# JihyongOh/DeMFI

Measured on AMD Instinct MI355X. Metric: interpolated frames/sec @720p x8 MFI (N_tst=3), higher is better.
Workload: dtype f16; 1 GPU; DeMFI-Net_rb N_tst=3, x8 MFI, 720x1280 (padded 736x1280), fp16, clip-parallel windows, random-init weights; uint8 frames host->HBM->host inside the timed region (PNG codec excluded), 8 distinct windows; graph=True, parallelism=clip1, n_ctx=7, n_trunk=3

## Files before the change

### demfi_amd/_lib.py

```python
import ctypes as C
import os

_HERE = os.path.dirname(os.path.abspath(__file__))
LIB_PATH = os.environ.get('DEMFI_HIP_LIB') or os.path.join(_HERE, 'csrc', 'libdemfi_hip.so')

F16, F32 = 0, 1
ABI_VERSION = 8
ACT_NONE, ACT_RELU, ACT_TANH, ACT_SIGMOID = 0, 1, 2, 3
MODE_STORE, MODE_MUL, MODE_GRU = 0, 1, 2
BT601, BT709 = 0, 1
SITING_420JPEG, SITING_420MPEG2 = 0, 1
YUV_LAYOUT = {'420': 0, '422': 1, '444': 2, 'mono': 3}
OWNERS = ('sep', 'wstream7', 'ws2', 'wstream3', 'c64', 'narrow_nhwc', 'narrow_thin', 'general')
OWNERS_COUT_PERM = frozenset(range(6))
MAX_PIECES, MAX_CHUNKS, MAX_SEGS, MAX_OCTS = 48, 40, 8, 32


class View(C.Structure):
    _fields_ = [('ptr', C.c_void_p), ('sx', C.c_int64), ('sy', C.c_int64), ('sc', C.c_int64), ('sb', C.c_int64),
                ('is_f32', C.c_int32), ('_pad', C.c_int32)]


class Piece(C.Structure):
    _fields_ = [('v', View), ('nch', C.c_int32), ('lds_ch', C.c_int32), ('up_shift', C.c_int32), ('fat', C.c_int32)]


class Chunk(C.Structure):
    _fields_ = [('first_piece', C.c_int32), ('n_pieces', C.c_int32), ('nks', C.c_int32), ('_pad', C.c_int32),
                ('w_off', C.c_int64)]


class Seg(C.Structure):
# ... 39 lines not shown


class Op(C.Structure):
    _fields_ = [('kind', C.c_int32), ('conv', C.c_int32), ('nch', C.c_int32), ('_pad', C.c_int32), ('macs', C.c_int64),
                ('a', View), ('b', View), ('o', View), ('p', C.c_void_p * 32), ('t', C.c_void_p), ('name', C.c_char * 64),
                ('bt', Batch)]


_SIGS = {
    'demfi_abi_version': (C.c_int, []),
    'demfi_last_error': (C.c_char_p, []),
    'demfi_device_info': (C.c_int, [C.c_char_p, C.c_int, C.POINTER(C.c_int), C.POINTER(C.c_int64)]),
    'demfi_pack_conv_weights': (C.c_int, [C.c_void_p, C.c_int, C.c_int, C.c_int, C.c_int, C.c_void_p, C.c_int,
                                          C.c_void_p, C.c_int, C.c_void_p, C.c_int, C.c_int, C.c_int, C.c_void_p,
                                          C.POINTER(C.c_int64)]),
    'demfi_conv_lds_bytes': (C.c_int64, [C.POINTER(Conv)]),
    'demfi_conv2d': (C.c_int, [C.POINTER(Conv), C.c_void_p, C.c_void_p]),
    'demfi_resblock_eligible': (C.c_int, [C.POINTER(Conv), C.POINTER(Conv)]),
    'demfi_resblock3x3_c64': (C.c_int, [C.POINTER(Conv), C.POINTER(Conv), C.c_void_p]),
    'demfi_gru_r_eligible': (C.c_int, [C.POINTER(Conv)]),
    'demfi_gru_r': (C.c_int, [C.POINTER(Conv), C.c_void_p]),
    'demfi_gru_zq_eligible': (C.c_int, [C.POINTER(Conv), C.POINTER(Conv)]),
    'demfi_gru_zq': (C.c_int, [C.POINTER(Conv), C.POINTER(Conv), C.c_void_p]),
    'demfi_space_to_depth': (C.c_int, [C.c_void_p, C.c_void_p, C.c_int, C.c_int, C.c_int, C.c_void_p]),
    'demfi_reflect_pad': (C.c_int, [C.c_void_p, C.c_void_p, C.c_int, C.c_int, C.c_int, C.c_int, C.c_int, C.c_void_p]),
    'demfi_overlay_mean': (C.c_int, [C.c_void_p, C.c_void_p, C.c_int, C.c_int, C.c_void_p]),
    'demfi_cfr_workspace_bytes': (C.c_int64, [C.c_int, C.c_int]),
    'demfi_cfr_reset': (C.c_int, [C.c_void_p, C.c_int, C.c_int, C.c_void_p]),
    'demfi_cfr_flow_align': (C.c_int, [C.c_void_p, C.c_void_p, C.c_void_p, C.c_int, C.c_int, C.c_void_p, C.c_void_p,
                                       C.c_void_p, C.c_void_p]),
    'demfi_warp_blend': (C.c_int, [C.POINTER(View), C.c_void_p, C.POINTER(View), C.c_void_p, C.c_void_p, C.c_void_p,
                                   C.POINTER(View), C.c_int, C.c_int, C.c_int, C.c_void_p, C.c_void_p, C.c_void_p]),
    'demfi_warp_blend_pack': (C.c_int, [C.POINTER(View), C.c_void_p, C.POINTER(View), C.c_void_p, C.c_void_p, C.c_void_p,
                                        C.POINTER(View), C.c_int, C.c_int, C.c_void_p, C.c_void_p, C.c_int, C.c_void_p]),
    'demfi_warp_blend_batched': (C.c_int, [C.POINTER(View), C.c_void_p, C.POINTER(View), C.c_void_p, C.c_void_p, C.c_void_p,
                                           C.POINTER(View), C.c_int, C.c_int, C.c_int, C.c_void_p, C.c_void_p, C.c_int, C.POINTER(Batch),
                                           C.c_void_p]),
    'demfi_cfr_flow_align_batched': (C.c_int, [C.c_void_p, C.c_void_p, C.c_void_p, C.c_int, C.c_int, C.c_void_p, C.c_void_p,
                                               C.POINTER(Batch), C.c_void_p]),
    'demfi_cfr_flow_align_pack': (C.c_int, [C.c_void_p, C.c_void_p, C.c_void_p, C.c_void_p, C.c_int, C.c_int, C.c_void_p, C.c_void_p, C.c_void_p,
                                            C.c_int, C.POINTER(Batch), C.c_void_p]),
    'demfi_pack_planes_batched': (C.c_int, [C.c_void_p, C.c_int, C.c_void_p, C.c_int, C.c_int64, C.c_int, C.c_int, C.POINTER(Batch),
                                            C.c_void_p]),
    'demfi_fgac_gather': (C.c_int, [C.POINTER(View), C.c_void_p, C.POINTER(View), C.c_int, C.c_int, C.c_int,
                                    C.c_void_p, C.c_void_p]),
    'demfi_fgac_window': (C.c_int, [C.POINTER(View), C.POINTER(View), C.c_void_p, C.POINTER(View), C.c_int, C.c_int, C.c_int,
# ... 146 lines not shown
```

### demfi_amd/csrc/conv_build.cpp

```cpp
#include "plan.h"
#include <algorithm>
#include <string.h>

namespace plan {

constexpr int64_t LDS_BUDGET = 78 * 1024;

int conv_shape(int dtype, int H, int W, int stride, int batch, const Layer& l, const demfi_conv_src* srcs, int n_srcs,
               const demfi_conv_dst* dsts, int n_dsts, ConvShape& out, const char* name, int pad_y, int pad_x, int grid_div)
{
    if (dtype != DEMFI_F16 && dtype != DEMFI_F32) return demfi_set_error(DEMFI_ERR_ARG, "%s: dtype", name);
    if (!srcs || !dsts || n_srcs <= 0 || n_dsts <= 0 || n_dsts > DEMFI_MAX_SEGS || (stride != 1 && stride != 2))
        return demfi_set_error(DEMFI_ERR_ARG, "%s: sources / destinations / stride", name);
    const int cout = l.cout, cin = l.cin, kh = l.kh, kw = l.kw;
    const int esz = dtype == DEMFI_F32 ? 4 : 2;
    const int64_t LH = 7 * stride + kh, LW = 31 * stride + kw;
    int n_oct = 0;
    for (int i = 0; i < n_dsts; ++i) n_oct += (dsts[i].n + 7) / 8;
    const int sub = (n_oct + 3) / 4;
    int nco = sub <= 5 ? sub : 4;
    int rec = 128;
    int src_nch = 0;
    for (int i = 0; i < n_srcs; ++i) src_nch += srcs[i].nch;
    const bool ws2_s2 = stride == 2 && kh == 4 && kw == 4, ws2_s1 = stride == 1 && kh == 3 && kw == 3 && src_nch > 64;
// ... 180 lines not shown
                pm[i] = cout_map[sb * 32 + (r >> 4) * 16 + ((r >> 2) & 1) * 8 + ((r >> 3) & 1) * 4 + (r & 3)];
            }
            cout_map.swap(pm);
        }
    }
    out.wbytes = d.w_blk_stride * 16 * (cout_pad / (32 * nco));
    return DEMFI_OK;
}

int conv_pack(const ConvShape& s, const Layer& l, const float* w, const float* bias, std::vector<uint8_t>& wpack, std::vector<float>& bias_packed)
{
    int64_t nbytes = 0;
    wpack.resize(s.wbytes);
    const int st = demfi_pack_conv_weights(w, l.cout, l.cin, l.kh, l.kw, s.cin_map.data(), (int)s.cin_map.size(), s.nks.data(), (int)s.nks.size(),
                                           s.cout_map.data(), s.d.cout_pad, s.d.nco, s.d.dtype, wpack.data(), &nbytes);
    if (st < 0) return st;
    if (nbytes != s.wbytes) return demfi_set_error(DEMFI_ERR_ARG, "conv_pack: %lld B packed, %lld B planned", (long long)nbytes, (long long)s.wbytes);
    bias_packed.assign(s.d.cout_pad, 0.0f);
    for (int i = 0; i < s.d.cout_pad; ++i)
        if (s.cout_map[i] >= 0 && bias) bias_packed[i] = bias[s.cout_map[i]];
    return DEMFI_OK;
}

}

extern "C" int demfi_conv_build(int dtype, int H, int W, int stride, int batch, const float* w, const float* bias, int cout, int cin,
                                int kh, int kw, const demfi_conv_src* srcs, int n_srcs, const demfi_conv_dst* dsts, int n_dsts,
                                demfi_conv* desc, void* wpack, int64_t* wpack_bytes, float* bias_packed, int32_t* cout_pad)
{
    if (!w || !desc || !wpack_bytes || !cout_pad || H <= 0 || W <= 0 || batch <= 0 || cout <= 0 || cin <= 0 || kh <= 0 || kw <= 0)
        return demfi_set_error(DEMFI_ERR_ARG, "demfi_conv_build: bad arguments");
    const plan::Layer l = {cout, cin, kh, kw};
    plan::ConvShape s;
    int st = plan::conv_shape(dtype, H, W, stride, batch, l, srcs, n_srcs, dsts, n_dsts, s, "demfi_conv_build");
    if (st < 0) return st;
    *cout_pad = s.d.cout_pad;
    *wpack_bytes = s.wbytes;
    *desc = s.d;
    if (!wpack) return DEMFI_OK;
    std::vector<uint8_t> wp;
    std::vector<float> bp;
    st = plan::conv_pack(s, l, w, bias, wp, bp);
    if (st < 0) return st;
    memcpy(wpack, wp.data(), wp.size());
    if (bias_packed) memcpy(bias_packed, bp.data(), bp.size() * 4);
    return DEMFI_OK;
// ... 2 lines not shown
```

### demfi_amd/csrc/conv_kernels.h

```cpp
#pragma once
#include <hip/hip_runtime.h>
#include "demfi_hip.h"

int demfi_conv_general_launch(const demfi_conv* h, const demfi_conv* dev, hipStream_t st, size_t lds);
int demfi_c64_launch(const demfi_conv* h, const demfi_conv* dev, hipStream_t st);
int demfi_narrow_launch(const demfi_conv* h, const demfi_conv* dev, hipStream_t st, bool thin);
bool demfi_sep_eligible(const demfi_conv* h);
int demfi_sep_launch(const demfi_conv* h, const demfi_conv* dev, hipStream_t st);
bool demfi_wstream_eligible(const demfi_conv* h, int ks = 7, int nch = 2);
int demfi_wstream_launch(const demfi_conv* h, const demfi_conv* dev, hipStream_t st);
int demfi_wstream3_launch(const demfi_conv* h, const demfi_conv* dev, hipStream_t st);
int demfi_c64_trace_collect(unsigned long long* acc);
int demfi_narrow_trace_collect(unsigned long long* acc);
int demfi_sep_trace_collect(unsigned long long* acc);
int demfi_wstream_trace_collect(unsigned long long* acc);
```

### demfi_amd/csrc/ctx.cpp

```cpp
#include "plan.h"
#include <stdlib.h>
#include <string.h>

using namespace plan;

namespace {

int run_ops(demfi_ctx* c, const OpList& ops, void* stream)
{
    for (const demfi_op& op : ops) {
        const int st = demfi_run_op(c, &op, stream);
        if (st < 0) return st;
    }
    return DEMFI_OK;
}

bool check_idx(const demfi_ctx* c, int trunk, int q)
{
    return c && trunk >= 0 && trunk < c->n_trunk && q >= 0 && q < c->n_ctx;
}

}

static int size_context(demfi_ctx* c, demfi_ctx** out)
{
    layer_table(c);
    compute_layout(c, 0, 0);
    int st = run_builder(c, true);
    if (st < 0) { delete c; return st; }
    static const bool arena_on = !(getenv("DEMFI_ARENA") && atoi(getenv("DEMFI_ARENA")) == 0);
    if (arena_on && !c->op_kind) {
        std::vector<const OpList*> per_t = {&c->head_ops[0][0]}, tr = {&c->tr_ops[0]}, none;
        for (int it = 0; it < c->N; ++it) per_t.push_back(&c->iter_ops[0][0][it]);
        std::vector<const OpList*> per_t_all = per_t;
        if (c->n_ctx > 1) { per_t_all.push_back(&c->tb_head_ops[0]); for (int it = 0; it < c->N; ++it) per_t_all.push_back(&c->tb_iter_ops[0][it]); }
        const ArenaPlan pt = plan_arena(c, c->t_bufs[0][0], c->n_ctx, per_t, none,
                                        {"Ft", "u1", "u2", "u3", "d0", "d1", "d2", "rF", "dec_a", "dec_t", "dec_b", "frec0", "frec1", "re1", "rd64", "de1",
                                         "bl1", "xb", "zb", "rh", "h1", "fo1", "g_a", "g_t", "g_b", "g_p2", "misc16", "ref16", "ref32", "agg3s"});
        const ArenaPlan ptr_ = plan_arena(c, c->tr_bufs[0], 0, tr, per_t_all,
                                          {"s2d", "f1", "x0", "grow", "gffcat", "g0", "g1", "up", "enc_a", "enc_t", "enc_b", "rk", "skk", "rkp", "skp",
                                           "smp", "E", "wg"});
        c->arena_t = pt;
        c->arena_tr = ptr_;
        if (getenv("DEMFI_ARENA_DEBUG")) {
            for (auto* pl : {&c->arena_t, &c->arena_tr}) {
                fprintf(stderr, "arena %s: %.1f MB\n", pl == &c->arena_t ? "per-t (all contexts)" : "trunk", pl->size / 1e6);
                for (auto& kv : pl->off) fprintf(stderr, "   %-8s at %.1f MB\n", kv.first.c_str(), kv.second / 1e6);
            }
        }
// ... 259 lines not shown
extern "C" int demfi_ctx_get_op(const demfi_ctx* c, int segment, int trunk, int q, int iter, int index, demfi_op* out)
{
    const OpList* o = seg_ops(c, segment, trunk, q, iter);
    if (!o || !out || index < 0 || index >= (int)o->size()) return demfi_set_error(DEMFI_ERR_ARG, "demfi_ctx_get_op: bad arguments");
    *out = (*o)[index];
    return DEMFI_OK;
}

extern "C" int demfi_ctx_num_convs(const demfi_ctx* c) { return c ? (int)c->descs.size() : 0; }

extern "C" const demfi_conv* demfi_ctx_conv_desc(const demfi_ctx* c, int index)
{
    if (!c || index < 0 || index >= (int)c->descs.size()) return nullptr;
    return &c->descs[index];
}

extern "C" int demfi_run_op(demfi_ctx* c, const demfi_op* op, void* stream)
{
    if (!c || !op || !c->bound || c->on_host) return demfi_set_error(DEMFI_ERR_ARG, "demfi_run_op: context not bound to device memory");
    const int H = c->H, W = c->W;
    switch (op->kind) {
    case DEMFI_OP_CONV:
        if (op->conv < 0 || op->conv >= (int)c->descs.size()) return demfi_set_error(DEMFI_ERR_ARG, "demfi_run_op: descriptor index");
        return demfi_conv2d(&c->descs[op->conv], (const demfi_conv*)(c->base + c->desc_off) + op->conv, stream);
    case DEMFI_OP_RESBLOCK:
        if (op->conv < 0 || op->conv >= (int)c->descs.size() || op->nch < 0 || op->nch >= (int)c->descs.size())
            return demfi_set_error(DEMFI_ERR_ARG, "demfi_run_op: descriptor index");
        return demfi_resblock3x3_c64(&c->descs[op->conv], &c->descs[op->nch], stream);
    case DEMFI_OP_GRU_R:
        if (op->conv < 0 || op->conv >= (int)c->descs.size()) return demfi_set_error(DEMFI_ERR_ARG, "demfi_run_op: descriptor index");
        return demfi_gru_r(&c->descs[op->conv], stream);
    case DEMFI_OP_GRU_ZQ:
        if (op->conv < 0 || op->conv >= (int)c->descs.size() || op->nch < 0 || op->nch >= (int)c->descs.size())
            return demfi_set_error(DEMFI_ERR_ARG, "demfi_run_op: descriptor index");
        return demfi_gru_zq(&c->descs[op->conv], &c->descs[op->nch], stream);
    case DEMFI_OP_PACK:
        if (op->bt.nb > 1)
            return demfi_pack_planes_batched((const float* const*)op->p, op->nch, op->o.ptr, c->dtype, op->o.sx, H, W, &op->bt, stream);
        return demfi_pack_planes((const float* const*)op->p, op->nch, op->o.ptr, c->dtype, op->o.sx, H, W, stream);
    case DEMFI_OP_VIZ:
        if (op->conv == 0) return demfi_absmean_map(&op->a, op->b.ptr ? &op->b : nullptr, (float*)op->p[0], op->nch, H, W, stream);
        if (op->conv == 1) return demfi_minmax_normalize((float*)op->p[0], (int64_t)H * W, (float*)op->p[1], stream);
        if (op->conv == 2) return demfi_one_minus((const float*)op->p[1], (float*)op->p[0], (int64_t)H * W, stream);
        return demfi_set_error(DEMFI_ERR_ARG, "demfi_run_op: visualisation sub-op %d", op->conv);
    case DEMFI_OP_S2D:
        return demfi_space_to_depth((const float*)op->p[0], (void*)op->p[1], c->dtype, H, W, stream);
// ... 32 lines not shown
```

### demfi_amd/csrc/plan.cpp

```cpp
#include "plan.h"
#include <algorithm>
#include <string.h>

namespace plan {

void layer_table(demfi_ctx* c)
{
    auto& t = c->table;
    if (c->op_kind == 1) {
        for (const char* g : {"z", "r", "q"}) t[std::string("conv") + g + "1"] = {64, 128, 1, 5};
        for (const char* g : {"z", "r", "q"}) t[std::string("conv") + g + "2"] = {64, 128, 5, 1};
        return;
    }
    if (c->op_kind == 2) {
        t["conv_ref_k"] = {64, 64, 1, 1}; t["conv_source_k"] = {64, 64, 1, 1}; t["fusion"] = {64, 64, 1, 1};
        t["w_gen"] = {64, 128, 3, 3}; t["w_gen_2"] = {1, 64, 3, 3};
        return;
    }
    const int nf = c->hp.nf, r2 = c->hp.scale_factor * c->hp.scale_factor;
    const int G0 = 96, G = 32, Cn = 4, D = 12;
    auto add = [&](const std::string& n, int cout, int cin, int kh, int kw) { t[n] = {cout, cin, kh, kw}; };
    std::string p = "FF_RDB_Module.";
    add(p + "SFENet1", G0, 12 * r2, 5, 5);
    add(p + "SFENet2", G0, G0, 3, 3);
// ... 611 lines not shown
                m2.insert(m2.end(), 7, -1);
                SubW wb = sub_weight(p + "enc1", sel, false);
                conv(th, p + "enc1#t", {fsrc(B["Ft"], 0), fsrc_map(B["misc16"], m2)},
                     {D(fview(B["u1"]), range(0, 64), R, DEMFI_MODE_STORE, fview(TB["u1a"]))}, H2, W2, ConvOpt().strided(2).weights(wb));
            } else
            conv(th, p + "enc1", {fsrc(aF, 0, 0, -1, 0), fsrc(aF, 64, 0, -1, 1), fsrc(B["Ft"], 128), fsrc_map(B["misc16"], m)},
                 {D(fview(B["u1"]), range(0, 64), R)}, H2, W2, ConvOpt().strided(2));
        }
        conv(th, p + "enc2", {fsrc(B["u1"], 0)}, {D(fview(B["u2"]), range(0, 128), R)}, H4, W4, ConvOpt().strided(2));
        conv(th, p + "enc3", {fsrc(B["u2"], 0)}, {D(fview(B["u3"]), range(0, 256), R)}, H8, W8, ConvOpt().strided(2));
        conv(th, p + "dec0", {fsrc(B["u3"], 0)}, {D(fview(B["d0"]), range(0, 256), R)}, H8, W8);
        conv(th, p + "dec1", {fsrc(B["d0"], 0, 0, -1, -1, 1), fsrc(B["u2"], 256)}, {D(fview(B["d1"]), range(0, 128), R)}, H4, W4);
        conv(th, p + "dec2", {fsrc(B["d1"], 0, 0, -1, -1, 1), fsrc(B["u1"], 128)}, {D(fview(B["d2"]), range(0, 64), R)}, H2, W2);
        if (c->dtype == DEMFI_F16) {
            Found f3;
            if (!lookup(p + "dec3", f3)) return;
            const Layer l3 = f3.l;
            auto phase_view = [&](demfi_view v, int dy, int dx) {
                const int64_t elt = v.is_f32 ? 4 : 2;
                v.ptr = (char*)v.ptr + ((int64_t)dy * v.sy + (int64_t)dx * v.sx) * elt;
                v.sx *= 2; v.sy *= 2;
                return v;
            };
            for (int dy = 0; dy < 2 && status >= 0; ++dy) {
                SubW wf2;
                wf2.shape = {10, l3.cin, 3, 3};
                for (int dx = 0; dx < 2 && status >= 0; ++dx) {
                    std::vector<float> w9e;
                    if (!dry) {
                        w9e.assign((size_t)l3.cout * l3.cin * 9, 0.0f);
                        for (int co = 0; co < l3.cout; ++co)
                            for (int ci = 0; ci < l3.cin; ++ci) {
                                const float* w9 = &(*f3.w)[((size_t)co * l3.cin + ci) * 9];
                                float* we = &w9e[((size_t)co * l3.cin + ci) * 9];
                                for (int ky = 0; ky < 3; ++ky)
                                    for (int kx = 0; kx < 3; ++kx) {
                                        const int a = dy == 0 ? (ky >= 1) : (ky >= 2), b = dx == 0 ? (kx >= 1) : (kx >= 2);
                                        we[(a + dy) * 3 + (b + dx)] += w9[ky * 3 + kx];
                                    }
                            }
                    }
                    const std::string nm = p + "dec3#p" + std::to_string(dy) + std::to_string(dx);
                    const Layer l9 = {l3.cout, l3.cin, 3, 3};
                    const SubW wa = rows(l9, &w9e, f3.b, 5, 64), wb = rows(l9, &w9e, f3.b, 69, 64), wf = rows(l9, &w9e, f3.b, 0, 5);
                    conv(th, nm + "a", {fsrc(B["d2"], 0)},
                         {D(phase_view(fview(B["rF"], 0, 0), dy, dx), range(0, 64), T, DEMFI_MODE_STORE, phase_view(fview(aF, 0, 0), dy, dx))},
                         H2, W2, ConvOpt().weights(wa));
                    conv(th, nm + "b", {fsrc(B["d2"], 0)},
                         {D(phase_view(fview(B["rF"], 0, 1), dy, dx), range(0, 64), T, DEMFI_MODE_STORE, phase_view(fview(aF, 0, 1), dy, dx))},
                         H2, W2, ConvOpt().weights(wb));
                    wf2.w.insert(wf2.w.end(), wf.w.begin(), wf.w.end());
                    wf2.b.insert(wf2.b.end(), wf.b.begin(), wf.b.end());
                }
                if (status >= 0) {
                    conv(th, p + "dec3#p" + std::to_string(dy) + "xf", {fsrc(B["d2"], 0)},
                         {D(phase_view(delta_v(0, 0), dy, 0), range(0, 4), DEMFI_ACT_NONE, DEMFI_MODE_STORE, phase_view(tview(B["ft"]), dy, 0)),
                          D(phase_view(delta_v(0, 4), dy, 0), {4}, DEMFI_ACT_NONE, DEMFI_MODE_STORE, phase_view(tview(ffo, 4), dy, 0)),
                          D(phase_view(delta_v(0, 0), dy, 1), range(5, 9), DEMFI_ACT_NONE, DEMFI_MODE_STORE, phase_view(tview(B["ft"]), dy, 1)),
                          D(phase_view(delta_v(0, 4), dy, 1), {9}, DEMFI_ACT_NONE, DEMFI_MODE_STORE, phase_view(tview(ffo, 4), dy, 1))},
                         H2, W2, ConvOpt().weights(wf2).packed(phase_view(fview(B["delta16"]), dy, 0), 0, 4, 16, 20));
                }
            }
        } else
        conv(th, p + "dec3", {fsrc(B["d2"], 0, 0, -1, -1, 1)},
             {D(fview(B["rF"], 0, 0), range(5, 69), T, DEMFI_MODE_STORE, fview(aF, 0, 0)),
              D(fview(B["rF"], 0, 1), range(69, 133), T, DEMFI_MODE_STORE, fview(aF, 0, 1)),
              D(delta_v(0, 0), range(0, 4), DEMFI_ACT_NONE, DEMFI_MODE_STORE, tview(B["ft"])),
              D(delta_v(0, 4), {4}, DEMFI_ACT_NONE, DEMFI_MODE_STORE, tview(ffo, 4))}, H, W);
        warp(th, "warp_fat", 64, fview(B["rF"], 0, 0), fview(B["rF"], 0, 1), fview(B["rF"], 0, 2), delta_p(0, 0), delta_p(0, 2),
             delta_p(0, 4), plane(B["occ"], 0), tp);
        conv(th, "Dec_first", {fsrc(B["rF"], 0)}, {D(fview(B["dec_a"]), range(0, 64), R)}, H, W, ConvOpt().batched(3));
        const Tensor* cur = resblocks(th, "Decoder_res", c->hp.num_resb_dec, B["dec_a"], B["dec_t"], B["dec_b"], H, W, 3);
        conv(th, "Dec_last1", {fsrc(*cur, 0)}, {D(fview(B["dec_t"]), range(0, 64), R)}, H, W, ConvOpt().batched(3));
// ... 158 lines not shown
```

### demfi_amd/csrc/plan.h

```cpp
#pragma once
#include "common.h"
#include <map>
#include <string>
#include <vector>

namespace plan {

struct Tensor {
    int64_t off = -1;
    int kind = 0;
    int d[4] = {0, 0, 0, 0};
    int64_t bytes = 0;
    int64_t cstride = 0;
    int id = 0;
};

struct ArenaPlan { std::map<std::string, int64_t> off; int64_t size = 0; int64_t cstride = 0; bool on = false; };

struct Weight { std::vector<float> data; std::vector<int64_t> shape; };

struct Layer { int cout, cin, kh, kw; };

typedef std::map<std::string, Tensor> BufSet;
typedef std::vector<demfi_op> OpList;

struct ConvShape {
    demfi_conv d;
    std::vector<int32_t> cin_map, cout_map, nks;
    int64_t wbytes = 0;
    int64_t macs = 0;
};

int conv_shape(int dtype, int H, int W, int stride, int batch, const Layer& l, const demfi_conv_src* srcs, int n_srcs,
               const demfi_conv_dst* dsts, int n_dsts, ConvShape& out, const char* name, int pad_y = -1, int pad_x = -1, int grid_div = 1);
int conv_pack(const ConvShape& s, const Layer& l, const float* w, const float* bias, std::vector<uint8_t>& wpack, std::vector<float>& bias_packed);

}

struct demfi_ctx {
    int H, W, N, dtype, n_trunk, n_ctx;
    int op_kind = 0, op_batch = 1;
    demfi_hparams hp;
    std::map<std::string, plan::Weight> weights;
    std::map<std::string, plan::Layer> table;
    int64_t w_region = 0, w_bytes = 0, desc_off = 0, zero_off = 0, total = 0, n_descs = 0;
    std::vector<plan::BufSet> tr_bufs;
    std::vector<std::vector<plan::BufSet>> t_bufs;
    std::vector<int64_t> id_cstride;
    plan::ArenaPlan arena_t, arena_tr;
    bool bound = false, on_host = false;
    char* base = nullptr;
    std::vector<demfi_conv> descs;
    std::vector<plan::OpList> tr_ops;
    std::vector<std::vector<plan::OpList>> head_ops;
    std::vector<std::vector<std::vector<plan::OpList>>> iter_ops;
    std::vector<plan::OpList> tb_head_ops;
    std::vector<std::vector<plan::OpList>> tb_iter_ops;
    std::vector<std::string> fused_dry, fused_now;
    std::vector<uint8_t> host_blob;
    std::map<std::string, std::pair<int64_t, int64_t>> pack_cache;
    int64_t blob_fill = 0;
};

// ... 12 lines not shown
```

### demfi_amd/engine.py

```python
import ctypes as C

import numpy as np
import torch

from . import _lib as L
from .spec import HyperParams


def _np_f32(t):
    return np.ascontiguousarray(t.detach().to('cpu', torch.float32).numpy())


class _Src:
    __slots__ = ('fat', 'ptr', 'sx', 'sy', 'sc', 'sb', 'is_f32', 'cin', 'up')

    def __init__(self, fat, ptr, sx, sy, sc, sb, is_f32, cin, up=0):
        self.fat, self.ptr, self.sx, self.sy, self.sc, self.sb = fat, ptr, sx, sy, sc, sb
        self.is_f32, self.cin, self.up = is_f32, list(cin), up


class _Dst:
    __slots__ = ('view', 'couts', 'act', 'mode', 'res', 'aux', 'scale', 'dy', 'dx')

    def __init__(self, view, couts, act=L.ACT_NONE, mode=L.MODE_STORE, res=None, aux=None, scale=1, dy=0, dx=0):
# ... 121 lines not shown
            host[off:off + a.nbytes] = a.reshape(-1)
        self.weight_blob = torch.from_numpy(host).to(self.device)
        self._wblobs = None
        base = self.weight_blob.data_ptr()
        self.zero_page = torch.zeros(256, dtype=torch.uint8, device=self.device)
        self._keep.append(self.zero_page)
        for d in self._descs:
            d.wpack = base + (d.wpack or 0)
            d.bias = base + (d.bias or 0)
            d.zero_page = self.zero_page.data_ptr()
        sz = C.sizeof(L.Conv)
        raw = bytearray(len(self._descs) * sz)
        for i, d in enumerate(self._descs):
            raw[i * sz:(i + 1) * sz] = bytes(d)
        self.desc_dev = torch.frombuffer(raw, dtype=torch.uint8).clone().to(self.device)
        self._desc_sz = sz

    def launch_conv(self, i, stream, what='conv'):
        L.check(self.lib.demfi_conv2d(C.byref(self._descs[i]), self.desc_dev.data_ptr() + i * self._desc_sz, stream), what)

    def launch_resblock(self, i1, i2, stream, what='resblock'):
        L.check(self.lib.demfi_resblock3x3_c64(C.byref(self._descs[i1]), C.byref(self._descs[i2]), stream), what)


    def launch_gru_r(self, i, stream, what='gru_r'):
        L.check(self.lib.demfi_gru_r(C.byref(self._descs[i]), stream), what)

    def launch_gru_zq(self, iz, iq, stream, what='gru_zq'):
        L.check(self.lib.demfi_gru_zq(C.byref(self._descs[iz]), C.byref(self._descs[iq]), stream), what)


SEG_TRUNK, SEG_HEAD, SEG_ITER, SEG_TB_HEAD, SEG_TB_ITER = 0, 1, 2, 3, 4
KIND_NAME = {0: 'conv', 1: 'pack', 2: 's2d', 3: 'overlay', 4: 'fgac', 5: 'gate', 6: 'cfr', 7: 'warp', 8: 'fgac_window', 9: 'avg_pool',
             10: 'resblock',
             11: 'gru_r', 12: 'gru_zq', 13: 'viz'}


class Engine:

    def __init__(self, state_dict, H, W, dtype=torch.float16, device='cuda:0', max_updates=3, hp=None, n_ctx=1, n_trunk=1):
        if H % 8 or W % 8:
            raise ValueError('DeMFI-Net needs H, W multiples of 8 (the harness pads to 32): got %dx%d' % (H, W))
        self.lib = L.load()
        self.H, self.W, self.N = H, W, max_updates
        self.dtype = dtype
        self.f32 = dtype == torch.float32
# ... 285 lines not shown
```

### include/demfi_hip.h

```cpp
#ifndef DEMFI_HIP_H
#define DEMFI_HIP_H

#include <stdint.h>

#ifdef __cplusplus
extern "C" {
#endif

#define DEMFI_ABI_VERSION 8

enum demfi_dtype { DEMFI_F16 = 0, DEMFI_F32 = 1 };

enum demfi_status {
    DEMFI_OK = 0,
    DEMFI_ERR_ARG = -1,
    DEMFI_ERR_HIP = -2,
    DEMFI_ERR_NODEV = -3
};

enum demfi_yuv_matrix { DEMFI_BT601 = 0, DEMFI_BT709 = 1 };
enum demfi_chroma_siting { DEMFI_420JPEG = 0, DEMFI_420MPEG2 = 1 };
enum demfi_yuv_layout { DEMFI_YUV_420 = 0, DEMFI_YUV_422 = 1, DEMFI_YUV_444 = 2, DEMFI_YUV_MONO = 3 };

enum demfi_act { DEMFI_ACT_NONE = 0, DEMFI_ACT_RELU = 1, DEMFI_ACT_TANH = 2, DEMFI_ACT_SIGMOID = 3 };
// ... 84 lines not shown
} demfi_u8_sink;

int         demfi_abi_version(void);
const char* demfi_last_error(void);
int         demfi_device_info(char* name, int len, int* n_cu, int64_t* hbm_bytes);

int demfi_pack_conv_weights(const float* w_oihw, int cout, int cin, int kh, int kw,
                            const int32_t* cin_map, int n_k, const int32_t* chunk_nks, int n_chunks,
                            const int32_t* cout_map, int cout_pad, int nco, int dtype,
                            void* out, int64_t* out_bytes);

int64_t demfi_conv_lds_bytes(const demfi_conv* host_desc);

int demfi_conv2d(const demfi_conv* host_desc, const demfi_conv* dev_desc, void* stream);

int demfi_resblock_eligible(const demfi_conv* h1, const demfi_conv* h2);
int demfi_resblock3x3_c64(const demfi_conv* h1, const demfi_conv* h2, void* stream);

int demfi_gru_r_eligible(const demfi_conv* hr);
int demfi_gru_r(const demfi_conv* hr, void* stream);
int demfi_gru_zq_eligible(const demfi_conv* hz, const demfi_conv* hq);
int demfi_gru_zq(const demfi_conv* hz, const demfi_conv* hq, void* stream);

int demfi_space_to_depth(const float* x, void* out, int dtype, int H, int W, void* stream);

int demfi_reflect_pad(const float* x, float* out, int planes, int h, int w, int H, int W, void* stream);

int demfi_overlay_mean(const float* x, float* out, int H, int W, void* stream);

int64_t demfi_cfr_workspace_bytes(int H, int W);
int demfi_cfr_reset(int64_t* acc, int H, int W, void* stream);
int demfi_cfr_flow_align(const float* flow01, const float* flow10, const float* t, int H, int W,
                         int64_t* acc, float* out, int32_t* dbg_idx, void* stream);

int demfi_warp_blend(const demfi_view* A, const float* fa, const demfi_view* B, const float* fb,
                     const float* logit, const float* t, const demfi_view* out, int C, int H, int W,
                     float* occ_out, int32_t* dbg_maps, void* stream);

int demfi_warp_blend_pack(const demfi_view* A, const float* fa, const demfi_view* B, const float* fb,
                          const float* logit, const float* t, const demfi_view* out, int H, int W, float* occ_out,
                          void* pack8, int pack_dtype, void* stream);

typedef struct demfi_batch {
    int32_t nb;
    int32_t _pad;
    int64_t a, b, o;
// ... 207 lines not shown
```

Measured before the change: 102.7 frames/s.

## Fuse dec3 upsample-conv phases into one warp-specialized onepass kernel

Adds a dedicated HIP kernel for the Refine_Module dec3 layer, a 3x3 conv over the x2 nearest-neighbour upsample of a 64-channel tensor. It computes all four sub-pixel phases and both 64-channel feature halves, adding the residual and applying tanh, in a single launch. Producer waves stream input windows into LDS with global_load_lds while MFMA waves compute from pre-packed per-phase weights, replacing eight separate phase convolutions that each re-read the input. It is enabled by default through an environment toggle, adds weight-packing code, and falls back when the layer is not eligible.

```diff
diff --git a/demfi_amd/_lib.py b/demfi_amd/_lib.py
--- a/demfi_amd/_lib.py
+++ b/demfi_amd/_lib.py
@@ -8,6 +8,7 @@
 ABI_VERSION = 8
 ACT_NONE, ACT_RELU, ACT_TANH, ACT_SIGMOID = 0, 1, 2, 3
 MODE_STORE, MODE_MUL, MODE_GRU = 0, 1, 2
+DEC3_WBYTES = 2 * 2 * 2 * 4 * 4 * 2 * 1024
 BT601, BT709 = 0, 1
 SITING_420JPEG, SITING_420MPEG2 = 0, 1
 YUV_LAYOUT = {'420': 0, '422': 1, '444': 2, 'mono': 3}
@@ -93,6 +94,9 @@
     'demfi_gru_r': (C.c_int, [C.POINTER(Conv), C.c_void_p]),
     'demfi_gru_zq_eligible': (C.c_int, [C.POINTER(Conv), C.POINTER(Conv)]),
     'demfi_gru_zq': (C.c_int, [C.POINTER(Conv), C.POINTER(Conv), C.c_void_p]),
+    'demfi_dec3_eligible': (C.c_int, [C.POINTER(Conv)]),
+    'demfi_dec3_onepass': (C.c_int, [C.POINTER(Conv), C.c_void_p, C.c_void_p, C.c_void_p]),
+    'demfi_dec3_pack': (C.c_int, [C.c_void_p, C.c_void_p, C.c_int, C.c_int, C.c_void_p, C.c_void_p]),
     'demfi_space_to_depth': (C.c_int, [C.c_void_p, C.c_void_p, C.c_int, C.c_int, C.c_int, C.c_void_p]),
     'demfi_reflect_pad': (C.c_int, [C.c_void_p, C.c_void_p, C.c_int, C.c_int, C.c_int, C.c_int, C.c_int, C.c_void_p]),
     'demfi_overlay_mean': (C.c_int, [C.c_void_p, C.c_void_p, C.c_int, C.c_int, C.c_void_p]),
diff --git a/demfi_amd/csrc/conv_build.cpp b/demfi_amd/csrc/conv_build.cpp
--- a/demfi_amd/csrc/conv_build.cpp
+++ b/demfi_amd/csrc/conv_build.cpp
@@ -226,6 +226,55 @@
     return DEMFI_OK;
 }
 
+void dec3_embed(const float* w, int cin, int co0, int n, int dy, int dx, std::vector<float>& w9e)
+{
+    w9e.assign((size_t)n * cin * 9, 0.0f);
+    for (int co = 0; co < n; ++co)
+        for (int ci = 0; ci < cin; ++ci) {
+            const float* w9 = w + ((size_t)(co0 + co) * cin + ci) * 9;
+            float* we = &w9e[((size_t)co * cin + ci) * 9];
+            for (int ky = 0; ky < 3; ++ky)
+                for (int kx = 0; kx < 3; ++kx) {
+                    const int a = dy == 0 ? (ky >= 1) : (ky >= 2), b = dx == 0 ? (kx >= 1) : (kx >= 2);
+                    we[(a + dy) * 3 + (b + dx)] += w9[ky * 3 + kx];
+                }
+        }
+}
+
+}
+
+extern "C" int demfi_dec3_pack(const float* w, const float* bias, int cout, int co0, void* wphase, float* bphase)
+{
+    if (!w || !bias || !wphase || !bphase || co0 < 0 || cout < co0 + 128)
+        return demfi_set_error(DEMFI_ERR_ARG, "demfi_dec3_pack: null argument, or rows [%d, %d) outside the %d of the layer", co0, co0 + 128, cout);
+    std::vector<int32_t> cin_map(64), cout_map(64);
+    for (int i = 0; i < 64; ++i) {
+        const int sb = i / 32, r = i % 32;
+        cin_map[i] = i;
+        cout_map[i] = sb * 32 + (r >> 4) * 16 + ((r >> 2) & 1) * 8 + ((r >> 3) & 1) * 4 + (r & 3);
+    }
+    const int32_t nks = 4;
+    std::vector<float> w9e;
+    std::vector<uint8_t> full(9 * 4 * 2 * 1024);
+    uint8_t* out = (uint8_t*)wphase;
+    for (int dy = 0; dy < 2; ++dy)
+        for (int dx = 0; dx < 2; ++dx)
+            for (int fh = 0; fh < 2; ++fh) {
+                plan::dec3_embed(w, 64, co0 + fh * 64, 64, dy, dx, w9e);
+                int64_t nbytes = 0;
+                const int st = demfi_pack_conv_weights(w9e.data(), 64, 64, 3, 3, cin_map.data(), 64, &nks, 1, cout_map.data(), 64, 2, DEMFI_F16,
+                                                       full.data(), &nbytes);
+                if (st < 0) return st;
+                if (nbytes != (int64_t)full.size()) return demfi_set_error(DEMFI_ERR_ARG, "demfi_dec3_pack: %lld B packed", (long long)nbytes);
+                for (int a = 0; a < 2; ++a)
+                    for (int b = 0; b < 2; ++b) {
+                        const int tap = (dy + a) * 3 + (dx + b);
+                        memcpy(out + ((((dy * 2 + dx) * 2 + fh) * 4 + (a * 2 + b)) * (int64_t)(4 * 2 * 1024)), full.data() + tap * (4 * 2 * 1024), 4 * 2 * 1024);
+                    }
+            }
+    for (int fh = 0; fh < 2; ++fh)
+        for (int i = 0; i < 64; ++i) bphase[fh * 64 + i] = bias[co0 + fh * 64 + cout_map[i]];
+    return DEMFI_OK;
 }
 
 extern "C" int demfi_conv_build(int dtype, int H, int W, int stride, int batch, const float* w, const float* bias, int cout, int cin,
diff --git a/demfi_amd/csrc/conv_kernels.h b/demfi_amd/csrc/conv_kernels.h
--- a/demfi_amd/csrc/conv_kernels.h
+++ b/demfi_amd/csrc/conv_kernels.h
@@ -10,6 +10,8 @@
 bool demfi_wstream_eligible(const demfi_conv* h, int ks = 7, int nch = 2);
 int demfi_wstream_launch(const demfi_conv* h, const demfi_conv* dev, hipStream_t st);
 int demfi_wstream3_launch(const demfi_conv* h, const demfi_conv* dev, hipStream_t st);
+extern "C" int demfi_dec3_eligible(const demfi_conv* h);
+extern "C" int demfi_dec3_onepass(const demfi_conv* h, const void* wphase, const float* bphase, void* stream);
 int demfi_c64_trace_collect(unsigned long long* acc);
 int demfi_narrow_trace_collect(unsigned long long* acc);
 int demfi_sep_trace_collect(unsigned long long* acc);
diff --git a/demfi_amd/csrc/ctx.cpp b/demfi_amd/csrc/ctx.cpp
--- a/demfi_amd/csrc/ctx.cpp
+++ b/demfi_amd/csrc/ctx.cpp
@@ -25,6 +25,7 @@
 static int size_context(demfi_ctx* c, demfi_ctx** out)
 {
     layer_table(c);
+    c->dec3_onepass = !(getenv("DEMFI_DEC3_ONEPASS") && atoi(getenv("DEMFI_DEC3_ONEPASS")) == 0);
     compute_layout(c, 0, 0);
     int st = run_builder(c, true);
     if (st < 0) { delete c; return st; }
@@ -330,6 +331,7 @@
     switch (op->kind) {
     case DEMFI_OP_CONV:
         if (op->conv < 0 || op->conv >= (int)c->descs.size()) return demfi_set_error(DEMFI_ERR_ARG, "demfi_run_op: descriptor index");
+        if (op->p[0]) return demfi_dec3_onepass(&c->descs[op->conv], op->p[0], (const float*)op->p[1], stream);
         return demfi_conv2d(&c->descs[op->conv], (const demfi_conv*)(c->base + c->desc_off) + op->conv, stream);
     case DEMFI_OP_RESBLOCK:
         if (op->conv < 0 || op->conv >= (int)c->descs.size() || op->nch < 0 || op->nch >= (int)c->descs.size())
diff --git a/demfi_amd/csrc/dec3.hip b/demfi_amd/csrc/dec3.hip
--- /dev/null
+++ b/demfi_amd/csrc/dec3.hip
@@ -0,0 +1,368 @@
+#include "kernel_kit.h"
+
+namespace {
+
+constexpr int D3_R = 8;
+constexpr int D3_CW = 32;
+constexpr int D3_IW = D3_CW + 2;
+constexpr int D3_IL = D3_R + 2;
+constexpr int D3_LS = D3_IW * 128;
+constexpr int D3_NI = (D3_IL * D3_IW + 7) / 8;
+constexpr int D3_WIN = D3_NI * 1024;
+constexpr int D3_STG_OFF = 2 * D3_WIN;
+constexpr int D3_STG = (D3_R / 2) * 2 * D3_CW * 256;
+constexpr int D3_BIAS_OFF = D3_STG_OFF + D3_STG;
+constexpr int D3_LDS = D3_BIAS_OFF + 128 * 4;
+constexpr int D3_NH = 4;
+constexpr int D3_NTHREADS = 256 + 64 * D3_NH;
+constexpr int D3_NIW = (D3_NI + D3_NH - 1) / D3_NH;
+constexpr int D3_NCH = D3_STG / 2048 / D3_NH;
+constexpr int D3_DEPTH = 4;
+constexpr int D3_NSTEP = 16;
+constexpr int D3_WBLK = 4 * 4 * 2 * 1024;
+static_assert(D3_NSTEP % D3_DEPTH == 0, "static ring indices");
+static_assert(D3_LDS <= 160 * 1024, "LDS budget");
+
+struct D3Args {
+    const char* src;  int64_t s_sx, s_sy, s_sb;
+    char* dst[2];     int64_t d_sx, d_sy, d_sb;
+    const char* res[2]; int64_t r_sx, r_sy, r_sb;
+    const char* w;
+    const float* bias;
+    const char* zeros;
+    int h, w_, batch;
+    int n_strips, n_rsteps;
+};
+
+__global__ __launch_bounds__(D3_NTHREADS, 1) void dec3_onepass_kernel(const D3Args a)
+{
+    extern __shared__ __attribute__((aligned(16))) char smem[];
+    const int tid = threadIdx.x;
+    const int lane = tid & 63;
+    const int wave = __builtin_amdgcn_readfirstlane(tid >> 6);
+    const int h = a.h, w = a.w_;
+    const int per_img = a.n_strips * a.n_rsteps;
+    const int total = per_img * a.batch;
+    int it0, it1;
+    XCD_ITEM_RUN(total, it0, it1);
+    if (it0 >= it1) return;
+    auto pos_of = [&](int it, int& img, int& x0, int& y0) {
+        const int rem = it / a.batch;
+        img = it - rem * a.batch;
+        const int strip = rem / a.n_rsteps;
+        x0 = strip * D3_CW;
+        y0 = (rem - strip * a.n_rsteps) * D3_R;
+    };
+
+    if (wave >= 4) {
+        const int dw = wave - 4;
+        __builtin_assume(dw >= 0 && dw < D3_NH);
+        unsigned off[D3_NIW];
+        int lc[D3_NIW];
+#pragma unroll
+        for (int k = 0; k < D3_NIW; ++k) {
+            const int i = dw + D3_NH * k;
+            const int rec = i * 8 + (lane >> 3);
+            const int rc = min(rec, D3_IL * D3_IW - 1);
+            const int l = rc / D3_IW, c = rc - l * D3_IW;
+            off[k] = (unsigned)(l * a.s_sy + c * a.s_sx) + (((lane & 7) ^ ((c >> 1) & 7)) << 4);
+            lc[k] = (i < D3_NI && rec < D3_IL * D3_IW) ? (l | (c << 8)) : 0xffff;
+        }
+        auto issue_window = [&](int it, int buf) {
+            int img, x0, y0;
+            pos_of(it, img, x0, y0);
+            const char* base = a.src + (int64_t)img * a.s_sb + (int64_t)(y0 - 1) * a.s_sy + (int64_t)(x0 - 1) * a.s_sx;
+            char* const wb = smem + buf * D3_WIN;
+            const bool interior = y0 >= 1 && y0 - 1 + D3_IL <= h && x0 >= 1 && x0 - 1 + D3_IW <= w;
+            if (interior) {
+#pragma unroll
+                for (int k = 0; k < D3_NIW; ++k) {
+                    const int i = dw + D3_NH * k;
+                    if (i >= D3_NI) continue;
+                    __builtin_amdgcn_global_load_lds((const DEMFI_GLOBAL void*)(base + off[k]),
+                                                     (__attribute__((address_space(3))) void*)(wb + i * 1024), 16, 0, 0);
+                }
+            } else {
+#pragma unroll
+                for (int k = 0; k < D3_NIW; ++k) {
+                    const int i = dw + D3_NH * k;
+                    if (i >= D3_NI) continue;
+                    const int iy = y0 - 1 + (lc[k] & 255), ix = x0 - 1 + (lc[k] >> 8);
+                    const char* g = (lc[k] != 0xffff && iy >= 0 && iy < h && ix >= 0 && ix < w) ? base + off[k] : a.zeros;
+                    __builtin_amdgcn_global_load_lds((const DEMFI_GLOBAL void*)g,
+                                                     (__attribute__((address_space(3))) void*)(wb + i * 1024), 16, 0, 0);
+                }
+            }
+        };
+        u4_t FA[D3_NCH][2], FB[D3_NCH][2];
+        const int spx = dw * 8 + (lane >> 3);
+        const unsigned dlane = (unsigned)(2 * spx * a.d_sx) + ((lane & 7) << 4);
+        const char* const sbp = smem + D3_STG_OFF + spx * 256;
+        const int sl0 = ((2 * (lane & 7)) ^ (spx & 15)) << 4, sl1 = ((2 * (lane & 7) + 1) ^ (spx & 15)) << 4;
+        auto stage_read = [&](u4_t (&F)[D3_NCH][2]) {
+#pragma unroll
+            for (int k = 0; k < D3_NCH; ++k) {
+                F[k][0] = *(const u4_t*)(sbp + (k >> 1) * 16384 + (k & 1) * 8192 + sl0);
+                F[k][1] = *(const u4_t*)(sbp + (k >> 1) * 16384 + (k & 1) * 8192 + sl1);
+            }
+            asm volatile("s_waitcnt lgkmcnt(0)" ::: "memory");
+        };
+        auto finish_store = [&](const u4_t (&F)[D3_NCH][2], int img, int x0, int y0, int dy, int fh, int hh) {
+            char* const obase = a.dst[fh] + (int64_t)img * a.d_sb + (int64_t)(2 * (y0 + 4 * hh) + dy) * a.d_sy + (int64_t)(2 * x0) * a.d_sx;
+            const bool px_ok = x0 + spx < w;
+#pragma unroll
+            for (int k = 0; k < D3_NCH; ++k) {
+                const f4_t f0 = __builtin_bit_cast(f4_t, F[k][0]), f1 = __builtin_bit_cast(f4_t, F[k][1]);
+                h8_t o;
+#pragma unroll
+                for (int j = 0; j < 4; ++j) {
+                    o[j] = (half_t)fast_tanh(f0[j]);
+                    o[4 + j] = (half_t)fast_tanh(f1[j]);
+                }
+                if (px_ok && y0 + 4 * hh + (k >> 1) < h)
+                    __builtin_nontemporal_store(__builtin_bit_cast(u4_t, o), gp<u4_t>(obase + (k >> 1) * 2 * a.d_sy + (k & 1) * a.d_sx + dlane));
+            }
+        };
+        issue_window(it0, 0);
+        asm volatile("s_waitcnt vmcnt(0)" ::: "memory");
+        asm volatile("s_barrier" ::: "memory");
+        int buf = 0;
+        for (int it = it0; it < it1; ++it, buf ^= 1) {
+            int img, x0, y0;
+            pos_of(it, img, x0, y0);
+            for (int blk = 0; blk < 4; ++blk) {
+                if (blk == 3) asm volatile("s_waitcnt vmcnt(0)" ::: "memory");
+                asm volatile("s_barrier" ::: "memory");
+                stage_read(FA);
+                asm volatile("s_barrier" ::: "memory");
+                asm volatile("s_barrier" ::: "memory");
+                stage_read(FB);
+                asm volatile("s_barrier" ::: "memory");
+                if (blk == 0 && it + 1 < it1) issue_window(it + 1, buf ^ 1);
+                finish_store(FA, img, x0, y0, blk >> 1, blk & 1, 0);
+                finish_store(FB, img, x0, y0, blk >> 1, blk & 1, 1);
+            }
+        }
+        return;
+    }
+
+    const int hi = lane >> 5, lx = lane & 31;
+    const int cs = wave & 1, dx = wave >> 1;
+    const unsigned lane16 = lane * 16;
+    if (dx == 0 && lane < 32) {
+        ((float*)(smem + D3_BIAS_OFF))[cs * 32 + lane] = a.bias[cs * 32 + lane];
+        ((float*)(smem + D3_BIAS_OFF))[64 + cs * 32 + lane] = a.bias[64 + cs * 32 + lane];
+    }
+    int boff0[2];
+#pragma unroll
+    for (int b = 0; b < 2; ++b) {
+        const int col = lx + dx + b;
+        boff0[b] = col * 128 + ((hi ^ ((col >> 1) & 7)) << 4);
+    }
+    auto boff = [&](auto G) {
+        constexpr int g = decltype(G)::value;
+        int b = boff0[g >> 2];
+        asm volatile("" : "+v"(b));
+        return b ^ ((g & 3) << 5);
+    };
+    int soff[2][2];
+#pragma unroll
+    for (int m2 = 0; m2 < 2; ++m2) {
+#pragma unroll
+        for (int e = 0; e < 2; ++e) soff[m2][e] = dx * 8192 + lx * 256 + ((((cs * 4 + m2 * 2 + hi) * 2 + e) ^ (lx & 15)) << 4);
+    }
+    auto a_load = [&](const char* wp, auto T) {
+        constexpr int t = decltype(T)::value;
+        constexpr int g = t >> 1, ta = t & 1, tb = g >> 2, ks = g & 3;
+        const char* wb = wp;
+        asm volatile("" : "+s"(wb));
+        unsigned l16 = lane16;
+        asm volatile("" : "+v"(l16));
+        return __builtin_bit_cast(uint4, *gcp<u4_t>(wb + (unsigned)((((ta * 2 + tb) * 4 + ks) * 2) * 1024 + l16)));
+    };
+    auto wblock = [&](int blk) { return a.w + ((((blk >> 1) * 2 + dx) * 2 + (blk & 1)) * D3_WBLK + cs * 1024); };
+    uint4 A[D3_DEPTH];
+    f16x_t acc[8];
+    {
+        const char* w0 = wblock(0);
+        static_for<0, D3_DEPTH>([&](auto T) { A[decltype(T)::value] = a_load(w0, T); });
+    }
+    asm volatile("s_waitcnt lgkmcnt(0)" ::: "memory");
+    asm volatile("s_barrier" ::: "memory");
+
+    int buf = 0;
+    for (int it = it0; it < it1; ++it, buf ^= 1) {
+        int img, x0, y0;
+        pos_of(it, img, x0, y0);
+        const int64_t rcol = (int64_t)(2 * min(x0 + lx, w - 1) + dx) * a.r_sx + cs * 64 + hi * 16;
+        for (int blk = 0; blk < 4; ++blk) {
+            const int dy = blk >> 1, fh = blk & 1;
+            const char* const wcur = wblock(blk);
+            const char* const wnxt = wblock((blk + 1) & 3);
+            const char* const tin = smem + buf * D3_WIN + dy * D3_LS;
+            const char* const rimg = a.res[fh] + (int64_t)img * a.r_sb + rcol;
+            auto res_row = [&](int p, u4_t (&r)[2]) {
+                const char* rp = rimg + (int64_t)(2 * min(y0 + p, h - 1) + dy) * a.r_sy;
+                r[0] = *gcp<u4_t>(rp);
+                r[1] = *gcp<u4_t>(rp + 32);
+            };
+            u4_t R[8][2];
+            res_row(0, R[0]);
+            res_row(1, R[1]);
+            f16x_t c0;
+#pragma unroll
+            for (int g = 0; g < 4; ++g) {
+                const f4_t q = *(const f4_t*)(smem + D3_BIAS_OFF + (fh * 64 + cs * 32 + g * 8 + hi * 4) * 4);
+#pragma unroll
+                for (int j = 0; j < 4; ++j) c0[g * 4 + j] = q[j];
+            }
+            {
+                uint4 B[9];
+                {
+                    const int o = boff(std::integral_constant<int, 0>{});
+                    static_for<0, 9>([&](auto L) { B[decltype(L)::value] = *(const uint4*)(tin + decltype(L)::value * D3_LS + o); });
+                }
+                __builtin_amdgcn_sched_barrier(0);
+                static_for<0, D3_NSTEP>([&](auto T_) {
+                    constexpr int t = decltype(T_)::value;
+                    constexpr int g = t >> 1, ta = t & 1;
+                    const uint4 av = A[t % D3_DEPTH];
+                    if constexpr (t + D3_DEPTH < D3_NSTEP) A[t % D3_DEPTH] = a_load(wcur, std::integral_constant<int, t + D3_DEPTH>{});
+                    else                                   A[t % D3_DEPTH] = a_load(wnxt, std::integral_constant<int, t + D3_DEPTH - D3_NSTEP>{});
+                    if constexpr (ta == 0 || g + 1 == 8) {
+                        static_for<0, 8>([&](auto P) {
+                            constexpr int p = decltype(P)::value;
+                            if constexpr (t == 0) Mma<half_t>::initc(acc[p], av, B[p], c0);
+                            else Mma<half_t>::run(acc[p], av, B[ta + p]);
+                        });
+                        __builtin_amdgcn_sched_group_barrier(0x008, 2, 0);
+                        __builtin_amdgcn_sched_group_barrier(0x020, 1, 0);
+                        __builtin_amdgcn_sched_group_barrier(0x008, 6, 0);
+                    } else {
+                        const int o = boff(std::integral_constant<int, g + 1>{});
+                        static_for<0, 8>([&](auto P) {
+                            constexpr int p = decltype(P)::value;
+                            Mma<half_t>::run(acc[p], av, B[1 + p]);
+                            B[p] = *(const uint4*)(tin + p * D3_LS + o);
+                        });
+                        B[8] = *(const uint4*)(tin + 8 * D3_LS + o);
+                        __builtin_amdgcn_sched_group_barrier(0x008, 1, 0);
+                        __builtin_amdgcn_sched_group_barrier(0x100, 1, 0);
+                        __builtin_amdgcn_sched_group_barrier(0x008, 1, 0);
+                        __builtin_amdgcn_sched_group_barrier(0x020, 1, 0);
+                        __builtin_amdgcn_sched_group_barrier(0x100, 1, 0);
+#pragma unroll
+                        for (int q = 0; q < 6; ++q) {
+                            __builtin_amdgcn_sched_group_barrier(0x008, 1, 0);
+                            __builtin_amdgcn_sched_group_barrier(0x100, 1, 0);
+                        }
+                        __builtin_amdgcn_sched_group_barrier(0x100, 1, 0);
+                    }
+                    __builtin_amdgcn_sched_barrier(0);
+                });
+            }
+            static_for<2, 8>([&](auto P) { res_row(decltype(P)::value, R[decltype(P)::value]); });
+            __builtin_amdgcn_sched_barrier(0);
+            char* const srow = smem + D3_STG_OFF;
+            auto stage_half = [&](auto HH) {
+                static_for<0, 4>([&](auto PR) {
+                    constexpr int pr = decltype(PR)::value, p = 4 * decltype(HH)::value + pr;
+#pragma unroll
+                    for (int m2 = 0; m2 < 2; ++m2) {
+                        float v[8];
+#pragma unroll
+                        for (int j = 0; j < 4; ++j) {
+                            v[j] = acc[p][(2 * m2) * 4 + j];
+                            v[4 + j] = acc[p][(2 * m2 + 1) * 4 + j];
+                        }
+                        const u4_t r = R[p][m2];
+#pragma unroll
+                        for (int q = 0; q < 4; ++q) {
+                            v[2 * q] = res_mix_lo(r[q], v[2 * q]);
+                            v[2 * q + 1] = res_mix_hi(r[q], v[2 * q + 1]);
+                        }
+                        const f4_t lo = {v[0], v[1], v[2], v[3]}, hi4 = {v[4], v[5], v[6], v[7]};
+                        *(f4_t*)(srow + pr * 16384 + soff[m2][0]) = lo;
+                        *(f4_t*)(srow + pr * 16384 + soff[m2][1]) = hi4;
+                    }
+                });
+                asm volatile("s_waitcnt lgkmcnt(0)" ::: "memory");
+            };
+            stage_half(std::integral_constant<int, 0>{});
+            asm volatile("s_barrier" ::: "memory");
+            asm volatile("s_barrier" ::: "memory");
+            stage_half(std::integral_constant<int, 1>{});
+            asm volatile("s_barrier" ::: "memory");
+            asm volatile("s_barrier" ::: "memory");
+        }
+    }
+}
+
+bool d3_args(const demfi_conv* h, D3Args& a)
+{
+    if (!h || h->dtype != DEMFI_F16 || h->stride != 1 || h->kh != 3 || h->kw != 3 || h->pad_y != 1 || h->pad_x != 1) return false;
+    if (!h->zero_page || h->inH != h->H || h->inW != h->W || (h->H & 1) || (h->W & 1) || h->batch < 1) return false;
+    if (h->pack.ptr || h->u8_sink) return false;
+    const demfi_view* v0 = nullptr;
+    int nch = 0;
+    for (int i = 0; i < h->n_pieces; ++i) {
+        const demfi_piece& p = h->pieces[i];
+        if (!p.v.ptr) { if (p.nch) return false; continue; }
+        if (!p.fat || p.up_shift != 1 || p.v.is_f32 || p.v.sc != 1 || p.v.sx != 64) return false;
+        if (!v0) v0 = &p.v;
+        if ((const char*)p.v.ptr != (const char*)v0->ptr + nch * 2 || p.v.sy != v0->sy || p.v.sb != v0->sb) return false;
+        nch += p.nch;
+    }
+    if (!v0 || nch != 64) return false;
+    if (h->n_segs != 2 || h->cout_pad < 128) return false;
+    for (int o = 0; o < h->cout_pad / 8; ++o) {
+        if (o >= 16) { if (h->oct_n[o]) return false; continue; }
+        if (h->oct_seg[o] != o / 8 || h->oct_n[o] != 8 || h->oct_ch[o] != 8 * (o % 8)) return false;
+    }
+    for (int s = 0; s < 2; ++s) {
+        const demfi_seg& g = h->segs[s];
+        if (g.mode != DEMFI_MODE_STORE || g.act != DEMFI_ACT_TANH || g.scale != 1 || g.dy || g.dx || g.aux.ptr) return false;
+        if (!g.dst.ptr || g.dst.is_f32 || g.dst.sc != 1 || !g.res.ptr || g.res.is_f32 || g.res.sc != 1) return false;
+        if (g.dst.sx != h->segs[0].dst.sx || g.dst.sy != h->segs[0].dst.sy || g.dst.sb != h->segs[0].dst.sb) return false;
+        if (g.res.sx != h->segs[0].res.sx || g.res.sy != h->segs[0].res.sy || g.res.sb != h->segs[0].res.sb) return false;
+        if (g.dst.sx < 64 || g.res.sx < 64) return false;
+        a.dst[s] = (char*)g.dst.ptr;
+        a.res[s] = (const char*)g.res.ptr;
+    }
+    const demfi_view &d = h->segs[0].dst, &r = h->segs[0].res;
+    a.src = (const char*)v0->ptr; a.s_sx = v0->sx * 2; a.s_sy = v0->sy * 2; a.s_sb = v0->sb * 2;
+    a.d_sx = d.sx * 2; a.d_sy = d.sy * 2; a.d_sb = d.sb * 2;
+    a.r_sx = r.sx * 2; a.r_sy = r.sy * 2; a.r_sb = r.sb * 2;
+    a.zeros = (const char*)h->zero_page;
+    a.h = h->H / 2; a.w_ = h->W / 2; a.batch = h->batch;
+    a.n_strips = (a.w_ + D3_CW - 1) / D3_CW;
+    a.n_rsteps = (a.h + D3_R - 1) / D3_R;
+    if (a.s_sy * 12 + a.s_sx * 40 >= (int64_t)1 << 31 || a.d_sy * 20 + a.d_sx * 80 >= (int64_t)1 << 31) return false;
+    if (a.s_sy < 0 || a.s_sx < 0 || a.d_sy < 0 || a.d_sx < 0 || a.r_sy < 0 || a.r_sx < 0) return false;
+    const int64_t total = (int64_t)a.n_strips * a.n_rsteps * a.batch;
+    return total > 0 && total < (int64_t)1 << 30;
+}
+
+}
+
+extern "C" int demfi_dec3_eligible(const demfi_conv* h)
+{
+    D3Args a;
+    return d3_args(h, a) ? 1 : 0;
+}
+
+extern "C" int demfi_dec3_onepass(const demfi_conv* h, const void* wphase, const float* bphase, void* stream)
+{
+    D3Args a;
+    if (!wphase || !bphase || !d3_args(h, a))
+        return demfi_set_error(DEMFI_ERR_ARG, "demfi_dec3_onepass: not the layer this kernel runs (3x3 over the x2 NN-upsample of one 64-channel fp16 NHWC "
+                                              "tensor, two 64-channel fp16 destinations with residual and tanh) or no phase weights");
+    a.w = (const char*)wphase;
+    a.bias = bphase;
+    const int64_t total = (int64_t)a.n_strips * a.n_rsteps * a.batch;
+    DEMFI_LDS_ATTR(dec3_onepass_kernel);
+    const int grid = total >= 256 ? 256 : (int)total;
+    hipLaunchKernelGGL(dec3_onepass_kernel, dim3(grid), dim3(D3_NTHREADS), D3_LDS, (hipStream_t)stream, a);
+    DEMFI_HIP_CHECK(hipGetLastError());
+    return DEMFI_OK;
+}
diff --git a/demfi_amd/csrc/plan.cpp b/demfi_amd/csrc/plan.cpp
--- a/demfi_amd/csrc/plan.cpp
+++ b/demfi_amd/csrc/plan.cpp
@@ -657,33 +657,53 @@
                 v.sx *= 2; v.sy *= 2;
                 return v;
             };
+            bool onepass = false;
+            if (c->dec3_onepass && l3.cin == 64 && l3.cout == 133) {
+                const SubW wfeat = rows(l3, f3.w, f3.b, 5, 128);
+                conv(th, p + "dec3", {fsrc(B["d2"], 0, 0, -1, -1, 1)},
+                     {D(fview(B["rF"], 0, 0), range(0, 64), T, DEMFI_MODE_STORE, fview(aF, 0, 0)),
+                      D(fview(B["rF"], 0, 1), range(64, 128), T, DEMFI_MODE_STORE, fview(aF, 0, 1))}, H, W, ConvOpt().weights(wfeat));
+                if (status < 0) return;
+                demfi_conv probe = c->descs.back();
+                if (dry) { static const char some = 0; probe.zero_page = &some; }
+                if (demfi_dec3_eligible(&probe)) {
+                    auto hit = c->pack_cache.find("Refine_Module.dec3|phase");
+                    int64_t w_off, b_off;
+                    if (hit != c->pack_cache.end()) { w_off = hit->second.first; b_off = hit->second.second; }
+                    else {
+                        std::vector<uint8_t> wp(DEMFI_DEC3_WBYTES);
+                        std::vector<float> bp(128);
+                        if (!dry) status = demfi_dec3_pack(f3.w->data(), f3.b->data(), l3.cout, 5, wp.data(), bp.data());
+                        if (status < 0) return;
+                        w_off = blob_put(wp.data(), DEMFI_DEC3_WBYTES);
+                        b_off = blob_put(bp.data(), 128 * 4);
+                        if (status < 0) return;
+                        c->pack_cache["Refine_Module.dec3|phase"] = {w_off, b_off};
+                    }
+                    th.back().p[0] = c->base + c->w_region + w_off;
+                    th.back().p[1] = c->base + c->w_region + b_off;
+                    c->fused_now.push_back("dec3:" + p + "dec3");
+                    onepass = true;
+                } else th.pop_back();
+            }
             for (int dy = 0; dy < 2 && status >= 0; ++dy) {
                 SubW wf2;
                 wf2.shape = {10, l3.cin, 3, 3};
                 for (int dx = 0; dx < 2 && status >= 0; ++dx) {
                     std::vector<float> w9e;
-                    if (!dry) {
-                        w9e.assign((size_t)l3.cout * l3.cin * 9, 0.0f);
-                        for (int co = 0; co < l3.cout; ++co)
-                            for (int ci = 0; ci < l3.cin; ++ci) {
-                                const float* w9 = &(*f3.w)[((size_t)co * l3.cin + ci) * 9];
-                                float* we = &w9e[((size_t)co * l3.cin + ci) * 9];
-                                for (int ky = 0; ky < 3; ++ky)
-                                    for (int kx = 0; kx < 3; ++kx) {
-                                        const int a = dy == 0 ? (ky >= 1) : (ky >= 2), b = dx == 0 ? (kx >= 1) : (kx >= 2);
-                                        we[(a + dy) * 3 + (b + dx)] += w9[ky * 3 + kx];
-                                    }
-                            }
-                    }
+                    if (!dry) dec3_embed(f3.w->data(), l3.cin, 0, l3.cout, dy, dx, w9e);
                     const std::string nm = p + "dec3#p" + std::to_string(dy) + std::to_string(dx);
                     const Layer l9 = {l3.cout, l3.cin, 3, 3};
-                    const SubW wa = rows(l9, &w9e, f3.b, 5, 64), wb = rows(l9, &w9e, f3.b, 69, 64), wf = rows(l9, &w9e, f3.b, 0, 5);
-                    conv(th, nm + "a", {fsrc(B["d2"], 0)},
-                         {D(phase_view(fview(B["rF"], 0, 0), dy, dx), range(0, 64), T, DEMFI_MODE_STORE, phase_view(fview(aF, 0, 0), dy, dx))},
-                         H2, W2, ConvOpt().weights(wa));
-                    conv(th, nm + "b", {fsrc(B["d2"], 0)},
-                         {D(phase_view(fview(B["rF"], 0, 1), dy, dx), range(0, 64), T, DEMFI_MODE_STORE, phase_view(fview(aF, 0, 1), dy, dx))},
-                         H2, W2, ConvOpt().weights(wb));
+                    const SubW wf = rows(l9, &w9e, f3.b, 0, 5);
+                    if (!onepass) {
+                        const SubW wa = rows(l9, &w9e, f3.b, 5, 64), wb = rows(l9, &w9e, f3.b, 69, 64);
+                        conv(th, nm + "a", {fsrc(B["d2"], 0)},
+                             {D(phase_view(fview(B["rF"], 0, 0), dy, dx), range(0, 64), T, DEMFI_MODE_STORE, phase_view(fview(aF, 0, 0), dy, dx))},
+                             H2, W2, ConvOpt().weights(wa));
+                        conv(th, nm + "b", {fsrc(B["d2"], 0)},
+                             {D(phase_view(fview(B["rF"], 0, 1), dy, dx), range(0, 64), T, DEMFI_MODE_STORE, phase_view(fview(aF, 0, 1), dy, dx))},
+                             H2, W2, ConvOpt().weights(wb));
+                    }
                     wf2.w.insert(wf2.w.end(), wf.w.begin(), wf.w.end());
                     wf2.b.insert(wf2.b.end(), wf.b.begin(), wf.b.end());
                 }
diff --git a/demfi_amd/csrc/plan.h b/demfi_amd/csrc/plan.h
--- a/demfi_amd/csrc/plan.h
+++ b/demfi_amd/csrc/plan.h
@@ -34,11 +34,13 @@
 int conv_shape(int dtype, int H, int W, int stride, int batch, const Layer& l, const demfi_conv_src* srcs, int n_srcs,
                const demfi_conv_dst* dsts, int n_dsts, ConvShape& out, const char* name, int pad_y = -1, int pad_x = -1, int grid_div = 1);
 int conv_pack(const ConvShape& s, const Layer& l, const float* w, const float* bias, std::vector<uint8_t>& wpack, std::vector<float>& bias_packed);
+void dec3_embed(const float* w, int cin, int co0, int n, int dy, int dx, std::vector<float>& w9e);
 
 }
 
 struct demfi_ctx {
     int H, W, N, dtype, n_trunk, n_ctx;
+    bool dec3_onepass = true;
     int op_kind = 0, op_batch = 1;
     demfi_hparams hp;
     std::map<std::string, plan::Weight> weights;
diff --git a/demfi_amd/engine.py b/demfi_amd/engine.py
--- a/demfi_amd/engine.py
+++ b/demfi_amd/engine.py
@@ -167,6 +167,16 @@
     def launch_resblock(self, i1, i2, stream, what='resblock'):
         L.check(self.lib.demfi_resblock3x3_c64(C.byref(self._descs[i1]), C.byref(self._descs[i2]), stream), what)
 
+
+    def dec3_phase(self, weight, bias, co0=0):
+        wnp, bnp = _np_f32(weight), _np_f32(bias)
+        wp, bp = np.empty(L.DEC3_WBYTES, np.uint8), np.zeros(128, np.float32)
+        L.check(self.lib.demfi_dec3_pack(wnp.ctypes.data, bnp.ctypes.data, wnp.shape[0], co0, wp.ctypes.data, bp.ctypes.data), 'dec3_pack')
+        self._dec3 = (self._add_blob(wp), self._add_blob(bp.view(np.uint8)))
+
+    def launch_dec3(self, i, stream, what='dec3'):
+        base = self.weight_blob.data_ptr()
+        L.check(self.lib.demfi_dec3_onepass(C.byref(self._descs[i]), base + self._dec3[0], base + self._dec3[1], stream), what)
 
     def launch_gru_r(self, i, stream, what='gru_r'):
         L.check(self.lib.demfi_gru_r(C.byref(self._descs[i]), stream), what)
diff --git a/include/demfi_hip.h b/include/demfi_hip.h
--- a/include/demfi_hip.h
+++ b/include/demfi_hip.h
@@ -130,6 +130,11 @@
 int demfi_gru_zq_eligible(const demfi_conv* hz, const demfi_conv* hq);
 int demfi_gru_zq(const demfi_conv* hz, const demfi_conv* hq, void* stream);
 
+#define DEMFI_DEC3_WBYTES (2 * 2 * 2 * 4 * 4 * 2 * 1024)
+int demfi_dec3_eligible(const demfi_conv* h);
+int demfi_dec3_onepass(const demfi_conv* h, const void* wphase, const float* bphase, void* stream);
+int demfi_dec3_pack(const float* w, const float* bias, int cout, int co0, void* wphase, float* bphase);
+
 int demfi_space_to_depth(const float* x, void* out, int dtype, int H, int W, void* stream);
 
 int demfi_reflect_pad(const float* x, float* out, int planes, int h, int w, int H, int W, void* stream);
```

Measured after the change: 103.1 frames/s (median of 6 runs). About the same (+0.4%).
